# xuanyi-fu/xynet

Measured on AMD Instinct MI355X. Metric: GiB/s device-resident WebSocket XOR-unmask, 64KiB frames, 1/2/4/8 GPUs, higher is better.
Workload: dtype u8; 1 GPU; config 3: 32768 x 64 KiB masked binary frames (H=14), one contiguous 2 GiB batch; decoder=lattice (k_stream_lattice), mode=fused (xyws_decode_stream: boundaries discovered on device), frames_per_gpu=32768, batch_bytes_per_gpu=2147942400, payload_bytes_per_gpu=2147483648, batch_copies=1, parallelism=shard-by-frame x1, no collective

## Files before the change

xynet_amd/csrc/xyws_lattice.h:

```cpp

constexpr uint64_t LAT_FMIN = 128;
constexpr uint64_t LAT_FMAX = 1ull << 40;
enum {
  LW_CNT = 0,
  LW_BRK = 2,
  LW_UNMASK = 3,
  LW_W = 4,
  LW_LOOPS = 5,
  LW_DPOL = 6,
  LW_EPOCH = 7,
  LW_REDIR = 8,
  LW_NBAIL_POL = 12,
  LW_NBAIL_HYP = 13,
  LW_NLOOP_A = 14,
  LW_NLOOP_B = 15,
  LW_RCARRY = 16,
  LW_STAT = 32
};
enum { LS_AGG = 1, LS_BRK = 3 };
constexpr uint32_t LAT_SLIST = 512;
constexpr uint32_t LAT_NOCLAIM = 0x7FFFFFFFu;
enum : uint64_t { RD_DONE = 0, RD_FULL = 1, RD_FROM = 2 };

template <uint32_t NT_, uint32_t SEG_>
struct lgeom {
  static constexpr uint32_t NT = NT_, SEG = SEG_;
  static constexpr uint32_t TMAX = SEG_ / LAT_FMIN + 3;
};
using G_LAT = lgeom<1024, 15 * 8 * 1024>;
using G_LAT5 = lgeom<1024, 15 * 5 * 1024>;
constexpr uint64_t LAT5_MIN_FRAME = 16384;
using G_LAT_SMALL = lgeom<64, 1024>;

static_assert(LW_DPOL == LW_DPOL_WORD && LW_EPOCH == LW_DPOL + 1 && LW_DPOL % 2 == 0, "one 16-byte granule");

template <class GA, class GB>
struct llay {
  static_assert(GA::NT == GB::NT, "one workgroup size");
  static constexpr uint32_t NT = GA::NT;
  static constexpr uint32_t SEG = GA::SEG > GB::SEG ? GA::SEG : GB::SEG;
  static constexpr uint32_t TMAX = GA::TMAX > GB::TMAX ? GA::TMAX : GB::TMAX;
};
template <class GL>
struct __attribute__((aligned(256))) lat_lds {
  cstate S0;
  uint64_t E, X0, F, kmax, c0, kbf, nseg;
  uint64_t gk;
  uint32_t na, cur, nxt, brk, quit, done_last, nsl, big, nogate;
  uint64_t sl_seg[LAT_SLIST], sl_k[LAT_SLIST];
  uint4 tab[GL::TMAX];
  alignas(256) uint8_t seg[GL::SEG + 48];
};

XYWS_DEV uint32_t lat_rel(uint64_t x, uint64_t ss) {
  if (x <= ss) return 0;
  const uint64_t d = x - ss;
  return d > 0xFFFFFFFFull ? 0xFFFFFFFFu : (uint32_t)d;
}

constexpr uint32_t LAT_GRP = 64;
XYWS_DEV uint64_t lat_grp_size(const run_params& P, uint64_t g) {
  const uint64_t a = g * LAT_GRP;
  return a >= P.nseg ? 0 : (P.nseg - a < LAT_GRP ? P.nseg - a : LAT_GRP);
}

XYWS_DEV uint64_t lat_advance(const run_params& P, uint64_t E, uint32_t lane) {
  const uint64_t w = uniform64(st_load(P.lat + LW_W));
  if (w >= P.nseg) return w;
  uint64_t w1 = w;
  {
    const uint64_t g0 = w / LAT_GRP, g = g0 + lane, gs = lat_grp_size(P, g);
    const bool full = !gs || st_load(P.lgrp + g) == gs;
    const uint64_t nf = __ballot(!full);
    const uint32_t c = nf ? (uint32_t)__builtin_ctzll(nf) : 64u;
    const uint64_t wg = (g0 + c) * LAT_GRP;
    if (wg > w1) w1 = wg < P.nseg ? wg : P.nseg;
  }
  if (w1 < P.nseg) {
    bool dec[4];
#pragma unroll
    for (uint32_t r = 0; r < 4; r++) {
      const uint64_t j = w1 + 4 * lane + r;
      dec[r] = j >= P.nseg || (st_load(P.lat + LW_STAT + j) >> 2) == E;
    }
    const uint32_t lc = !dec[0] ? 0u : !dec[1] ? 1u : !dec[2] ? 2u : !dec[3] ? 3u : 4u;
    const uint64_t nd = __ballot(lc < 4);
    uint64_t w2 = w1 + 256;
    if (nd) {
      const uint32_t f = (uint32_t)__builtin_ctzll(nd);
      w2 = w1 + 4 * f + (uint32_t)__shfl((int)lc, (int)f, 64);
    }
    w1 = w2 < P.nseg ? w2 : P.nseg;
  }
  if (w1 > w && lane == 0) __hip_atomic_fetch_max(P.lat + LW_W, w1, __ATOMIC_RELAXED, __HIP_MEMORY_SCOPE_AGENT);
  return w1;
}
XYWS_DEV void lat_wait_decided(const run_params& P, uint64_t E, uint64_t s, uint32_t lane) {
  for (uint32_t it = 0; lat_advance(P, E, lane) <= s; it++) {
    if (it >= (1u << 20)) {
      if (lane == 0) atomicOr(P.head + 1, 2u);
      return;
    }
    __builtin_amdgcn_s_sleep(8);
  }
}

XYWS_DEV u32x4 lat_mask(const uint4* tab, uint32_t nent, uint32_t idx, uint32_t a) {
  const uint4 g = tab[idx];
  if (g.x <= a && a + 16u <= g.y) return u32x4{g.z, g.z, g.z, g.z};
  u32x4 m = span_key16(a, g.x, g.y, g.z);
  if (idx + 1 < nent) {
    const uint4 n = tab[idx + 1];
    if (n.x < a + 16u) m |= span_key16(a, n.x, n.y, n.z);
  }
  return m;
}

XYWS_DEV hdr_info lat_hdr(const run_params& P, const uint8_t* seg, uint32_t xr, uint64_t x) {
  const uint32_t* q = reinterpret_cast<const uint32_t*>(seg + (xr & ~3u));
  const uint32_t sh = xr & 3u, r0 = q[0], r1 = q[1], r2 = q[2], r3 = q[3], r4 = q[4];
  uint32_t w[4];
  w[0] = __builtin_amdgcn_alignbyte(r1, r0, sh);
  w[1] = __builtin_amdgcn_alignbyte(r2, r1, sh);
  w[2] = __builtin_amdgcn_alignbyte(r3, r2, sh);
  w[3] = __builtin_amdgcn_alignbyte(r4, r3, sh);
  const uint64_t room = P.hi - x;
  return parse_header_words(w, room < 16 ? (uint32_t)room : 16u);
}

XYWS_DEV __amdgpu_buffer_rsrc_t lat_rsrc(const run_params& P, uint64_t ss, uint32_t n) {
  const uint64_t top = (P.hi + 15) & ~15ull;
  const uint64_t room = top > ss ? top - ss : 0;
  return __builtin_amdgcn_make_buffer_rsrc(P.base + ss, 0, room < n ? (uint32_t)room : n, 0x00020000);
}

XYWS_DEV void write_frame(const run_params& P, uint64_t ord, uint64_t start, const hdr_info& h, uint64_t ps,
                          int32_t hdr_shift);

XYWS_DEV void lat_carried_frame(const run_params& P, const xyws_carry* cz) {
  if (!P.frames || !P.cap || cz->payload_remaining || !cz->hdr_len) return;
  const hdr_info hh = header_carried(P, cz);
  if (hh.hlen) write_frame(P, 0, P.lo, hh, P.lo + (hh.hlen - cz->hdr_len), (int32_t)cz->hdr_len);
}

template <class LL>
XYWS_DEV void lat_finish(const run_params& P, LL& L) {
  uint64_t* rd = P.lat + LW_REDIR;
  const xyws_carry* cz = P.cin_user ? P.cin_user : &k_zero_carry;
  {
    const uint32_t w = L.na == 2 ? LW_NBAIL_POL : L.na ? LW_NBAIL_HYP : L.big ? LW_NLOOP_A : LW_NLOOP_B;
    st_store(P.lat + w, st_load(P.lat + w) + 1);
  }
  if (L.na) {
    st_store(rd, RD_FULL);
  } else {
    const uint64_t b = st_load(P.lat + LW_BRK);
    const uint64_t X0 = L.X0, F = L.F, kmax = L.kmax, c0 = L.c0;
    lat_carried_frame(P, cz);
    if (b) {
      const uint64_t kb = ~b;
      const uint64_t tb = c0 + kb;
      uint64_t* rc = P.lat + LW_RCARRY;
#pragma unroll
      for (int i = 0; i < 8; i++) st_store(rc + i, 0);
      st_store(rc + 2, cz->frames_total + tb);
      st_store(rd + 1, X0 + kb * F);
      st_store(rd + 2, tb);
      st_store(rd, RD_FROM);
    } else {
      const uint64_t xl = X0 + (kmax - 1) * F;
      const hdr_info h = hdr_global(P, xl, NONE);
      uint64_t total = c0 + kmax;
      cstate S;
      if (!h.hlen) {
        S.X = xl; S.cov_ps = xl; S.cov_start = xl; S.cov_kw = 0; S.cov_key = 0; S.st = S_PARTIAL | S_NOCOV; S.pad = 0;
        total--;
      } else {
        S = frame_state(xl, h);
      }
      xyws_carry cinc;
#pragma unroll
      for (int i = 0; i < 8; i++) reinterpret_cast<uint64_t*>(&cinc)[i] = reinterpret_cast<const uint64_t*>(cz)[i];
      write_outputs(P, &cinc, total, S);
      dpol_publish(P, F, DEC_LATTICE);
      if (P.pol) {
        const uint64_t v[5] = {L.E, P.hi - P.lo, F, F, DEC_LATTICE};
#pragma unroll
        for (int i = 1; i < 5; i++) __hip_atomic_store(P.pol + i, v[i], __ATOMIC_RELAXED, __HIP_MEMORY_SCOPE_SYSTEM);
        __hip_atomic_store(P.pol, v[0], __ATOMIC_RELEASE, __HIP_MEMORY_SCOPE_SYSTEM);
      }
      st_store(rd, RD_DONE);
    }
  }
  uint32_t* cnt = reinterpret_cast<uint32_t*>(P.lat + LW_CNT);
  st_store(P.lat + LW_BRK, 0);
  st_store(P.lat + LW_W, 0);
  st_store(P.lat + LW_LOOPS, 0);
  __hip_atomic_store(cnt, 0u, __ATOMIC_RELAXED, __HIP_MEMORY_SCOPE_AGENT);
  __hip_atomic_store(cnt + 1, 0u, __ATOMIC_RELAXED, __HIP_MEMORY_SCOPE_AGENT);
  st_store(P.lat + LW_EPOCH, L.E);
}

XYWS_DEV bool lat_redirect(run_params& P) {
  if (!(P.opts & XYWS_OPT_REDIRECT)) return true;
  const uint64_t* r = P.lat + LW_REDIR;
  const uint64_t st = uniform64(st_load(r));
  if (st == RD_DONE) return false;
  if (st != RD_FROM) return true;
  const uint64_t p = uniform64(st_load(r + 1)), tb = uniform64(st_load(r + 2));
  const uint64_t pal = p & ~15ull;
  P.obias = p - P.lo;
  P.base += pal;
  P.lo = p - pal;
  P.hi -= pal;
  const uint64_t seg = P.segb, nseg = (P.hi + seg - 1) / seg, maxr = P.nruns;
  P.rbytes = nseg <= maxr ? seg : ((P.hi + maxr - 1) / maxr + 15) & ~15ull;
  P.nruns = (uint32_t)((P.hi + P.rbytes - 1) / P.rbytes);
  P.nflat = 2 * P.nruns;
  P.cin_user = reinterpret_cast<const xyws_carry*>(P.lat + LW_RCARRY);
  P.tbias = tb;
  if (P.frames) {
    const uint64_t c = P.cap < tb ? P.cap : tb;
    P.frames += c;
    P.cap -= c;
  }
  return true;
}

template <class G>
struct lat_io {
  static constexpr bool CTRL = G::NT >= 256;
  static constexpr uint32_t NW = G::NT / 64, NDW = CTRL ? NW - 1 : NW;
  static constexpr uint32_t NROW = G::SEG / 1024, K = (NROW + NDW - 1) / NDW;
  static constexpr uint32_t CLAIM = CTRL ? 64u : 0u;
  static_assert(G::SEG % 1024 == 0, "segments are whole 1 KiB rows");
  XYWS_DEV static bool data_wave(uint32_t wave) { return !CTRL || wave != 0; }
  XYWS_DEV static uint32_t row(uint32_t wave, uint32_t k) { return (CTRL ? wave - 1 : wave) + NDW * k; }
  XYWS_DEV static bool valid(uint32_t wave, uint32_t k) { return K * NDW == NROW || row(wave, k) < NROW; }
};

XYWS_DEV uint64_t lat_load_late(const uint64_t* p) {
  uint64_t v;
  asm volatile("global_load_dwordx2 %0, %1, off sc1" : "=v"(v) : "v"(p) : "memory");
  return v;
}

constexpr uint32_t LAT_NREP = 64, LAT_REPW = 32;
inline constexpr uint64_t lat_rep_off(uint64_t segs) {
  return (LW_STAT + segs + segs / 64 + 1 + LAT_REPW - 1) / LAT_REPW * LAT_REPW;
}
inline constexpr uint64_t lat_sl_off(uint64_t segs) { return lat_rep_off(segs) + LAT_NREP * LAT_REPW; }
XYWS_DEV void lat_raise_brk(const run_params& P, uint64_t k, uint32_t lane) {
  uint64_t o = 0;
  if (lane == 0) o = __hip_atomic_fetch_max(P.lat + LW_BRK, ~k, __ATOMIC_RELAXED, __HIP_MEMORY_SCOPE_AGENT);
  if (uniform64(o) >= ~k) return;
  __hip_atomic_fetch_max(P.lbrk + LAT_REPW * lane, ~k, __ATOMIC_RELAXED, __HIP_MEMORY_SCOPE_AGENT);
  asm volatile("s_waitcnt vmcnt(0)" ::: "memory");
}

XYWS_DEV uint32_t lat_ctrl_load(const run_params& P, uint64_t s, uint64_t SEGB, uint64_t X0, uint64_t F, uint64_t kmax,
                                uint32_t tid) {
  const uint64_t ss = s * SEGB;
  const uint64_t ka = ss <= X0 ? 0 : (ss - X0 + F - 1) / F;
  const uint64_t xc = ka && ka <= kmax ? X0 + (ka - 1) * F : ss;
  const uint64_t top = (P.hi + 3) & ~3ull;
  const uint32_t lane = tid & 63u;
  const bool pd = lane < 4;
  uint64_t q = (pd ? ss + SEGB : xc & ~3ull) + (uint32_t)(pd ? 4u * lane : 4u * (lane - 4u));
  if (q + 4 > top) q = top - 4;
  return __builtin_nontemporal_load(reinterpret_cast<const uint32_t*>(P.base + q));
}

enum { LR_ALL = 0, LR_CTRL = 1, LR_DATA = 2 };
enum { LT_C_A = 16, LT_C_C, LT_C_ADV, LT_D_FILL, LT_D_WB, LT_D_TAB, LT_D_WC, LT_D_MASK, LT_D_WD, LT_D_ST, LT_D_WA,
       LT_SEGS, LT_GATE, LT_END };
struct lat_clock {
  bool on;
  uint64_t t, acc[16];
  XYWS_DEV void start(bool o) {
    on = o;
    for (int i = 0; i < 16; i++) acc[i] = 0;
    t = on ? __builtin_amdgcn_s_memtime() : 0;
  }
  XYWS_DEV void mark(int slot) {
    if (!on) return;
    const uint64_t n = __builtin_amdgcn_s_memtime();
    acc[slot - 16] += n - t;
    t = n;
  }
  XYWS_DEV void flush(const run_params& P) {
    if (!on) return;
    for (int i = 0; i < 16; i++)
      if (acc[i]) stat_add(P, 16 + i, acc[i]);
  }
};
template <class G, int ROLE, class LL>
XYWS_DEV void lat_loop(const run_params& P, LL& L, uint32_t tid0, uint32_t ahead) {
  using IO = lat_io<G>;
  constexpr bool CT = ROLE != LR_DATA, DT = ROLE != LR_CTRL;
  uint32_t tid = tid0;
  asm volatile("" : "+v"(tid));
  const uint32_t lane = tid & 63u;
  const uint32_t wave = __builtin_amdgcn_readfirstlane(tid >> 6);
  uint32_t* cnt = reinterpret_cast<uint32_t*>(P.lat + LW_CNT);
  const uint64_t E = uniform64(L.E);
  const uint64_t X0 = uniform64(L.X0), F = uniform64(L.F), kmax = uniform64(L.kmax);
  const float rF = 1.0f / (float)(F < (1ull << 24) ? F : (1ull << 24));
  const uint32_t F32 = F < 0x80000000ull ? (uint32_t)F : 0x80000000u;
  uint32_t cur = uniform32(L.cur);
  uint32_t it = 0, nsl = 0;
  lat_clock clk;
  clk.start(stats_on(P) && (tid == 0 || (tid == 64 && DT)));
  uint64_t brk_seen = 0;
  const bool cl = tid == 0 && CT;
  u32x4 e[DT ? IO::K : 1];
  uint32_t cx = 0;
  constexpr uint32_t CW = IO::CLAIM / 64u;
  auto issue = [&](uint32_t s, bool claim, bool rows) {
    if constexpr (DT) {
      if (wave == CW) {
        if (lane == 0) {
          if (claim)
            asm volatile("global_atomic_add %0, %1, %2, off sc0" : "=v"(ahead) : "v"(cnt), "v"(1u) : "memory");
          else
            ahead = LAT_NOCLAIM;
        }
        cx = lat_ctrl_load(P, s, G::SEG, X0, F, kmax, tid);
      }
      if (rows) {
        const __amdgpu_buffer_rsrc_t rs = lat_rsrc(P, (uint64_t)s * G::SEG, G::SEG);
#pragma unroll
        for (uint32_t k = 0; k < IO::K; k++)
          e[k] = __builtin_amdgcn_raw_buffer_load_b128(rs, IO::valid(wave, k) ? lane * 16u : OOB,
                                                       IO::row(wave, k) * 1024u, AUX_NT);
      }
    }
  };
  if (DT && cur != NONE32) {
    const uint32_t a0 = ahead;
    issue(cur, false, true);
    ahead = a0;
    const __amdgpu_buffer_rsrc_t rs = lat_rsrc(P, (uint64_t)cur * G::SEG, G::SEG);
#pragma unroll
    for (uint32_t k = 0; k < IO::K; k++)
      __builtin_amdgcn_raw_buffer_store_b128(u32x4{0u, 0u, 0u, 0u}, rs, OOB, k * 1024u, AUX_ST_STREAM);
  }
  const uint32_t dl = IO::CTRL ? tid - 64u : tid, NDL = IO::NDW * 64u;
  while (cur != NONE32) {
    asm volatile("" : "+v"(tid));
    const uint64_t ss = (uint64_t)cur * G::SEG;
    const uint64_t se = ss + G::SEG;
    const uint64_t ka = ss <= X0 ? 0 : (ss - X0 + F - 1) / F;
    clk.mark(cl ? LT_C_ADV : LT_D_ST);
    __syncthreads();
    clk.mark(cl ? LT_C_ADV : LT_D_WA);
    if constexpr (DT) {
#pragma unroll
      for (uint32_t k = 0; k < IO::K; k++)
        if (IO::valid(wave, k)) *reinterpret_cast<u32x4*>(&L.seg[IO::row(wave, k) * 1024u + lane * 16u]) = e[k];
      if (clk.on) asm volatile("s_waitcnt lgkmcnt(0)" ::: "memory");
    }
    if (DT && wave == CW) {
      asm volatile("" : "+v"(ahead), "+v"(cx) : "v"(e[IO::K - 1].x));
      const uint32_t ln = tid & 63u;
      if (ln < 9) *reinterpret_cast<uint32_t*>(&L.seg[G::SEG + 4u * ln]) = cx;
      if (lane == 0) {
        const uint32_t a = ahead + 2u * gridDim.x;
        L.nxt = a < P.nseg ? a : NONE32;
        L.brk = NONE32;
      }
    }
    clk.mark(cl ? LT_C_A : LT_D_FILL);
    __syncthreads();
    clk.mark(cl ? LT_C_A : LT_D_WB);
    const uint32_t nxt = uniform32(L.nxt);
    uint64_t kz = se <= X0 ? 0 : (se - X0 + F - 1) / F;
    if (kz > kmax) kz = kmax;
    const uint32_t nl = kz > ka ? (uint32_t)(kz - ka) : 0u;
    if constexpr (DT) {
      if (tid == IO::CLAIM) {
        uint4 c = {0u, 0u, 0u, 0u};
        if (ka == 0) {
          const cstate S0 = L.S0;
          if (!(S0.st & S_NOCOV)) c = uint4{lat_rel(S0.cov_ps, ss), lat_rel(X0, ss), S0.cov_kw, 0u};
        } else if (ka <= kmax) {
          const uint64_t xc = X0 + (ka - 1) * F;
          const uint32_t sh = (uint32_t)(xc & 3);
          uint32_t w[4];
          const uint32_t* cw = reinterpret_cast<const uint32_t*>(&L.seg[G::SEG + 16]);
#pragma unroll
          for (int i = 0; i < 4; i++) w[i] = __builtin_amdgcn_alignbyte(cw[i + 1], cw[i], sh);
          const uint64_t room = P.hi - xc;
          const hdr_info h = parse_header_words(w, room < 16 ? (uint32_t)room : 16u);
          if (h.hlen) {
            const uint64_t ps = xc + h.hlen;
            const uint64_t end = ka == kmax ? sat_add(ps, h.plen) : xc + F;
            c = uint4{lat_rel(ps, ss), lat_rel(end < P.hi ? end : P.hi, ss), aligned_key(h.key, ps, 0), 0u};
          }
        }
        L.tab[0] = c;
      }
      if (nxt != NONE32) issue(nxt, !L.quit, true);
      const uint32_t nlw = (P.opts & XYWS_OPT_LATX_NOWORK) ? 0u : nl;
      for (uint32_t i = dl; i < nlw; i += NDL) {
        const uint64_t k = ka + i;
        const uint64_t x = X0 + k * F;
        const uint32_t xr = (uint32_t)(x - ss);
        const hdr_info h = lat_hdr(P, L.seg, xr, x);
        const bool last = k + 1 == kmax;
        const uint64_t fend = h.hlen ? sat_add(x + h.hlen, h.plen) : x;
        const bool ok = h.hlen ? ((uint64_t)h.hlen + h.plen == F && h.plen < F) || (last && fend >= P.hi) : last;
        if (!ok) atomicMin(&L.brk, i);
        uint4 en = {xr, xr, 0u, 0u};
        if (h.hlen) {
          const uint64_t ps = x + h.hlen;
          en = uint4{lat_rel(ps, ss), lat_rel(fend < P.hi ? fend : P.hi, ss), aligned_key(h.key, ps, 0), 0u};
        }
        L.tab[1 + i] = en;
      }
    }
    if (CT && tid == 0) {
      asm volatile("s_waitcnt vmcnt(0)" : "+v"(brk_seen)::"memory");
      if (cl) clk.mark(LT_GATE);
      L.gk = brk_seen;
    }
    clk.mark(cl ? LT_C_A : LT_D_TAB);
    __syncthreads();
    clk.mark(cl ? LT_C_C : LT_D_WC);
    const uint32_t brk = uniform32(L.brk);
    const bool blind = (P.opts & XYWS_OPT_TEST_LATSPEC) != 0;
    const bool gate = it == 0 && !blind && !(P.opts & XYWS_OPT_LAT_NOGATE);
    if (CT && tid < 64) {
      const uint64_t gk = uniform64(L.gk);
      if (brk != NONE32 && !(gk && ~gk <= ka + brk)) lat_raise_brk(P, ka + brk, lane);
      if (tid == 0) {
        st_store(P.lat + LW_STAT + cur, (E << 2) | (brk != NONE32 ? LS_BRK : LS_AGG));
        __hip_atomic_fetch_add(P.lgrp + cur / LAT_GRP, 1ull, __ATOMIC_RELAXED, __HIP_MEMORY_SCOPE_AGENT);
      }
      if (gate) {
        const uint64_t tg = clk.on ? __builtin_amdgcn_s_memtime() : 0;
        lat_wait_decided(P, E, cur, lane);
        if (tg && tid == 0) stat_add(P, LT_END, __builtin_amdgcn_s_memtime() - tg);
        if (tid == 0) L.gk = st_load(P.lat + LW_BRK);
      }
      if (tid == 0) brk_seen = lat_load_late(P.lbrk + LAT_REPW * (blockIdx.x % LAT_NREP));
    }
    if (gate) __syncthreads();
    clk.mark(cl ? LT_C_C : LT_D_WD);
    const uint64_t b = blind ? 0 : uniform64(L.gk);
    uint64_t kst = brk != NONE32 ? ka + brk : kz;
    if (b && ~b < kst) kst = ~b;
    uint32_t stop = kst >= kz ? G::SEG : lat_rel(X0 + kst * F, ss);
    if (stop > G::SEG) stop = G::SEG;
    bool quit = b || brk != NONE32;
    if (stop && !gate) {
      if (nsl < LAT_SLIST) {
        if (tid == IO::CLAIM) {
          L.sl_seg[nsl] = cur;
          L.sl_k[nsl] = kst;
        }
        nsl++;
      } else {
        const uint64_t k0 = ka ? ka - 1 : 0;
        if (tid == IO::CLAIM)
          for (uint32_t r = 0; r <= LAT_NREP; r++)
            __hip_atomic_fetch_max(r < LAT_NREP ? P.lbrk + LAT_REPW * r : P.lat + LW_BRK, ~k0, __ATOMIC_RELAXED,
                                   __HIP_MEMORY_SCOPE_AGENT);
        if (k0 < kst) {
          stop = lat_rel(X0 + k0 * F, ss);
          kst = k0;
        }
        quit = true;
      }
    }
    if (quit && tid == IO::CLAIM) L.quit = 1;
    if constexpr (DT) {
      const uint32_t xka = ka < kmax ? lat_rel(X0 + ka * F, ss) : 0xFFFFFFFFu;
      const uint32_t nent = brk != NONE32 ? 1u + brk : 1u + nl;
      const uint32_t lo_r = lat_rel(P.lo, ss), hi_r = P.hi - ss < G::SEG ? (uint32_t)(P.hi - ss) : G::SEG;
      const __amdgpu_buffer_rsrc_t rs = lat_rsrc(P, ss, G::SEG);
      const bool any = !(P.opts & XYWS_OPT_NO_STORE);
      const bool work = !(P.opts & XYWS_OPT_LATX_NOWORK);
      uint32_t edge = 0;
      u32x4 dprev = {0u, 0u, 0u, 0u};
#pragma unroll
      for (uint32_t k = 0; k < IO::K; k++) {
        const bool ok = IO::valid(wave, k);
        const uint32_t a = (ok ? IO::row(wave, k) : 0u) * 1024u + lane * 16u;
        u32x4 d = *reinterpret_cast<const u32x4*>(&L.seg[a]);
        uint32_t idx = 0;
        if (a >= xka) {
          const uint32_t dd = a - xka;
          uint32_t qq = (uint32_t)((float)dd * rF);
          if (qq * F32 > dd) qq--;
          else if ((qq + 1) * F32 <= dd) qq++;
          idx = 1 + qq;
        }
        if (work && idx < nent) d = d ^ lat_mask(L.tab, nent, idx, a);
        const bool whole = ok && a >= lo_r && a + 16u <= hi_r && a + 16u <= stop;
        if (ok && !whole && a < stop && a < hi_r && a + 16u > lo_r) {
          edge |= 1u << k;
          *reinterpret_cast<u32x4*>(&L.seg[a]) = d;
        }
        __builtin_amdgcn_raw_buffer_store_b128(d, rs, (whole && any) ? lane * 16u : OOB, IO::row(wave, k) * 1024u,
                                               AUX_ST_STREAM);
        asm volatile("" ::"v"(dprev.x), "v"(dprev.y), "v"(dprev.z), "v"(dprev.w));
        dprev = d;
      }
      asm volatile("s_nop 1" ::"v"(dprev.x), "v"(dprev.y), "v"(dprev.z), "v"(dprev.w));
#pragma nounroll
      while (edge && any) {
        const uint32_t k = __builtin_ctz(edge);
        edge &= edge - 1;
        const uint32_t a = IO::row(wave, k) * 1024u + lane * 16u;
#pragma nounroll
        for (uint32_t y = a; y < a + 16u; y++)
          if (y >= lo_r && y < hi_r && y < stop) P.base[ss + y] = L.seg[y];
      }
      if (P.frames && stop && kst > ka) {
        const uint32_t nd = (uint32_t)(kst - ka < nl ? kst - ka : nl);
        for (uint32_t i = dl; i < nd; i += NDL) {
          const uint64_t k = ka + i;
          const uint64_t ord = L.c0 + k;
          if (ord >= P.cap) break;
          const uint64_t x = X0 + k * F;
          const hdr_info h = lat_hdr(P, L.seg, (uint32_t)(x - ss), x);
          if (h.hlen) write_frame(P, ord, x, h, x + h.hlen, 0);
        }
      }
    }
    it++;
    if (clk.on && cl) clk.acc[LT_SEGS - 16]++;
    cur = nxt;
  }
  clk.mark(cl ? LT_C_ADV : LT_D_ST);
  clk.flush(P);
  if (DT && tid == IO::CLAIM) L.nsl = nsl;
}

constexpr uint32_t LAT_LSW = 1 + 2 * LAT_SLIST;
template <class G, class LL>
XYWS_DEV void lat_dump_list(const run_params& P, const LL& L, uint32_t tid) {
  const uint32_t n = L.nsl;
  uint64_t* q = P.lsl + (uint64_t)blockIdx.x * LAT_LSW;
  if (tid == 0) q[0] = n;
  for (uint32_t i = tid; i < n; i += G::NT) {
    q[1 + 2 * i] = L.sl_seg[i];
    q[2 + 2 * i] = L.sl_k[i];
  }
}

template <class G, class LL>
XYWS_DEV void lat_undo(const run_params& P, const LL& L, uint32_t tid, uint64_t s, uint64_t kst, uint64_t kb) {
  const uint64_t X0 = L.X0, F = L.F, kmax = L.kmax;
  const uint64_t ss = s * G::SEG;
  const uint32_t stop = (uint32_t)(X0 + kst * F - ss < G::SEG ? X0 + kst * F - ss : G::SEG);
  const uint32_t lo_r = lat_rel(P.lo, ss), hi_r = P.hi - ss < G::SEG ? (uint32_t)(P.hi - ss) : G::SEG;
  const uint32_t top = stop < hi_r ? stop : hi_r;
  const uint32_t from = lat_rel(X0 + kb * F, ss);
  for (uint32_t a = (from & ~15u) + tid * 16u; a < top; a += G::NT * 16u) {
    uint64_t g = a + ss < X0 ? NONE : (a + ss - X0) / F;
    u32x4 m = {0u, 0u, 0u, 0u};
    for (int t = 0; t < 2; t++, g = g == NONE ? 0 : g + 1) {
      uint4 en = {0u, 0u, 0u, 0u};
      if (g == NONE) {
        const cstate S0 = L.S0;
        if (!(S0.st & S_NOCOV)) en = uint4{lat_rel(S0.cov_ps, ss), lat_rel(X0, ss), S0.cov_kw, 0u};
      } else if (g < kst && g < kmax) {
        const uint64_t x = X0 + g * F;
        const hdr_info h = hdr_global(P, x, NONE);
        if (h.hlen) {
          const uint64_t ps = x + h.hlen;
          const uint64_t end = g + 1 == kmax ? sat_add(ps, h.plen) : x + F;
          en = uint4{lat_rel(ps, ss), lat_rel(end < P.hi ? end : P.hi, ss), aligned_key(h.key, ps, 0), 0u};
        }
      }
      m |= span_key16(a, en.x, en.y, en.z);
    }
    if (a >= from && a >= lo_r && a + 16u <= top) {
      uint32_t* q = reinterpret_cast<uint32_t*>(P.base + ss + a);
      const uint32_t mm[4] = {m.x, m.y, m.z, m.w};
#pragma unroll
      for (int i = 0; i < 4; i++) {
        if (!mm[i]) continue;
        const uint32_t v = __hip_atomic_load(q + i, __ATOMIC_RELAXED, __HIP_MEMORY_SCOPE_AGENT);
        __hip_atomic_store(q + i, v ^ mm[i], __ATOMIC_RELAXED, __HIP_MEMORY_SCOPE_AGENT);
      }
      continue;
    }
#pragma unroll
    for (uint32_t b = 0; b < 16; b++) {
      const uint32_t y = a + b;
      const uint32_t mw = b < 4 ? m.x : b < 8 ? m.y : b < 12 ? m.z : m.w;
      const uint8_t kbyte = (uint8_t)(mw >> (8u * (b & 3u)));
      if (kbyte && y >= from && y >= lo_r && y < top) {
        uint8_t* q = P.base + ss + y;
        const uint8_t v = __hip_atomic_load(q, __ATOMIC_RELAXED, __HIP_MEMORY_SCOPE_AGENT);
        __hip_atomic_store(q, (uint8_t)(v ^ kbyte), __ATOMIC_RELAXED, __HIP_MEMORY_SCOPE_AGENT);
      }
    }
  }
}

constexpr uint32_t LAT_UNDO_POLLS = 2048;

template <class G, class LL>
XYWS_DEV void lat_body(const run_params& P, LL& L, uint32_t tid, uint32_t ahead) {
  using IO = lat_io<G>;
  uint32_t* cnt = reinterpret_cast<uint32_t*>(P.lat + LW_CNT);
  if (!L.na) {
    if constexpr (IO::CTRL) {
      if (__builtin_amdgcn_readfirstlane(tid >> 6) == 0)
        lat_loop<G, LR_CTRL>(P, L, tid, ahead);
      else
        lat_loop<G, LR_DATA>(P, L, tid, ahead);
    } else {
      lat_loop<G, LR_ALL>(P, L, tid, ahead);
    }
    __syncthreads();
    if (tid < 64) {
      uint64_t b = 0;
      if (tid == 0) __hip_atomic_fetch_add(P.lat + LW_LOOPS, 1ull, __ATOMIC_RELAXED, __HIP_MEMORY_SCOPE_AGENT);
      if (L.quit && L.nsl) {
        const uint32_t polls = (P.opts & XYWS_OPT_TEST_LATDUMP) ? 0u : LAT_UNDO_POLLS;
        bool ended = false;
        for (uint32_t it = 0; it < polls; it++) {
          if (uniform64(st_load(P.lat + LW_LOOPS)) >= gridDim.x) {
            ended = true;
            break;
          }
          __builtin_amdgcn_s_sleep(8);
        }
        if (ended) b = uniform64(st_load(P.lat + LW_BRK));
      }
      if (tid == 0) L.kbf = b && L.nsl ? ~b : NONE;
    }
    __syncthreads();
    const uint64_t kb = L.kbf;
    if (kb != NONE) {
      const uint32_t n = L.nsl;
      for (uint32_t j = 0; j < n; j++)
        if (kb < L.sl_k[j]) lat_undo<G>(P, L, tid, L.sl_seg[j], L.sl_k[j], kb);
      asm volatile("s_waitcnt vmcnt(0)" ::: "memory");
      __syncthreads();
      if (tid == 0) L.nsl = 0;
      __syncthreads();
    }
    lat_dump_list<G>(P, L, tid);
  }
  asm volatile("s_waitcnt vmcnt(0)" ::: "memory");
  __syncthreads();
  if (tid == 0) {
    __builtin_amdgcn_fence(__ATOMIC_RELEASE, "agent");
    asm volatile("s_waitcnt vmcnt(0)" ::: "memory");
    const uint32_t last = atomicAdd(cnt + 1, 1u) + 1 == gridDim.x ? 1u : 0u;
    if (last) {
      __builtin_amdgcn_fence(__ATOMIC_ACQUIRE, "agent");
      asm volatile("s_waitcnt vmcnt(0)" ::: "memory");
    }
    L.done_last = last;
  }
  __syncthreads();
  if (!L.done_last) return;
  if (tid == 0) {
    const uint64_t b = st_load(P.lat + LW_BRK);
    L.kbf = b && !L.na ? ~b : NONE;
  }
  __syncthreads();
  const uint64_t kb = L.kbf;
  if (kb != NONE) {
    if (tid == 0) L.nsl = 0;
    __syncthreads();
    for (uint32_t w = tid; w < gridDim.x; w += G::NT) {
      const uint64_t* q = P.lsl + (uint64_t)w * LAT_LSW;
      const uint32_t n = (uint32_t)st_load(q);
      for (uint32_t i = 0; i < n; i++) {
        const uint64_t kst = st_load(q + 2 + 2 * i);
        if (kb < kst) {
          const uint32_t j = atomicAdd(&L.nsl, 1u);
          if (j < LAT_SLIST) {
            L.sl_seg[j] = st_load(q + 1 + 2 * i);
            L.sl_k[j] = kst;
          }
        }
      }
    }
    __syncthreads();
    const uint32_t nu = L.nsl;
    if (nu <= LAT_SLIST) {
      for (uint32_t j = 0; j < nu; j++) lat_undo<G>(P, L, tid, L.sl_seg[j], L.sl_k[j], kb);
    } else {
      for (uint32_t w = 0; w < gridDim.x; w++) {
        const uint64_t* q = P.lsl + (uint64_t)w * LAT_LSW;
        const uint32_t n = (uint32_t)st_load(q);
        for (uint32_t i = 0; i < n; i++) {
          const uint64_t kst = st_load(q + 2 + 2 * i);
          if (kb < kst) lat_undo<G>(P, L, tid, st_load(q + 1 + 2 * i), kst, kb);
        }
      }
    }
    asm volatile("s_waitcnt vmcnt(0)" ::: "memory");
    __syncthreads();
  }
  for (uint64_t g = tid; g * LAT_GRP < P.nseg; g += G::NT)
    __hip_atomic_store(P.lgrp + g, 0ull, __ATOMIC_RELAXED, __HIP_MEMORY_SCOPE_AGENT);
  if (tid < LAT_NREP) __hip_atomic_store(P.lbrk + LAT_REPW * tid, 0ull, __ATOMIC_RELAXED, __HIP_MEMORY_SCOPE_AGENT);
  if (tid != 0) return;
  lat_finish(P, L);
}

template <class GA, class GB>
__global__ void __launch_bounds__(GB::NT)
__attribute__((amdgpu_waves_per_eu(GB::NT >= 256 ? GB::NT / 256 : 1))) k_stream_lattice(run_params P0) {
  using GL = llay<GA, GB>;
  using IO = lat_io<GB>;
  static_assert(lat_io<GA>::CLAIM == IO::CLAIM, "one claim lane");
  extern __shared__ __attribute__((aligned(256))) uint8_t xs_lds[];
  lat_lds<GL>& L = *reinterpret_cast<lat_lds<GL>*>(xs_lds);
  const uint32_t tid = threadIdx.x;
  uint32_t ahead = NONE32;
  if (tid == 0) {
    const xyws_carry* cz = P0.cin_user ? P0.cin_user : &k_zero_carry;
    carry_words cc;
    uint32_t r0[5];
    uint64_t dp, ep;
    {
      u32x4 g;
      asm volatile("global_load_dwordx4 %0, %1, off sc1" : "=v"(g) : "v"(P0.lat + LW_DPOL) : "memory");
#pragma unroll
      for (int i = 0; i < 8; i++) cc.w[i] = reinterpret_cast<const uint64_t*>(cz)[i];
      const uint64_t a0 = P0.lo & ~3ull, dl = (P0.hi + 3) & ~3ull;
#pragma unroll
      for (int i = 0; i < 5; i++) {
        const uint64_t q = a0 + 4 * i;
        r0[i] = *reinterpret_cast<const uint32_t*>(P0.base + (q < dl ? q : dl - 4));
      }
      asm volatile("s_waitcnt vmcnt(0)" : "+v"(g)::"memory");
#pragma unroll
      for (int i = 0; i < 5; i++)
        if (a0 + 4 * i >= dl) r0[i] = 0u;
      dp = (uint64_t)g.x | ((uint64_t)g.y << 32);
      ep = (uint64_t)g.z | ((uint64_t)g.w << 32);
    }
    L.E = ep + 1;
    const bool dvalid = dp >> 63, dreg = (dp & ((1ull << 48) - 1)) >= LAT_FMIN;
    const uint64_t ddec = (dp >> 48) & 0x7Fu;
    uint32_t na = dvalid && !dreg && !(P0.opts & XYWS_OPT_LATTICE) ? 2u : 0u;
    L.nogate = dvalid && dreg && ddec == DEC_LATTICE && !(P0.opts & XYWS_OPT_LAT_GATE) ? 1u : 0u;
    uint64_t c0 = 0;
    const cstate S0 = initial_state_w(P0, cc, c0);
    if (!na && ((S0.st & S_PARTIAL) || S0.X >= P0.hi)) na = 1u;
    uint64_t F = 0, kmax = 0;
    if (!na) {
      hdr_info h;
      if (S0.X == P0.lo) {
        const uint32_t sh = (uint32_t)(P0.lo & 3);
        uint32_t w[4];
#pragma unroll
        for (int i = 0; i < 4; i++) w[i] = __builtin_amdgcn_alignbyte(r0[i + 1], r0[i], sh);
        const uint64_t room = P0.hi - P0.lo;
        h = parse_header_words(w, room < 16 ? (uint32_t)room : 16u);
      } else {
        h = hdr_global(P0, S0.X, NONE);
      }
      F = sat_add(h.hlen, h.plen);
      if (!h.hlen || F < LAT_FMIN || F > LAT_FMAX) na = 1;
      else kmax = (P0.hi - S0.X + F - 1) / F;
    }
    if (!na && kmax > 1 && !(P0.opts & (XYWS_OPT_TEST_LATSPEC | XYWS_OPT_LATX_NOCHK))) {
      const uint64_t dl = (P0.hi + 3) & ~3ull;
      uint32_t r[2][5];
#pragma unroll
      for (int j = 0; j < 2; j++) {
        const uint64_t a = (S0.X + (j + 1) * F) & ~3ull;
#pragma unroll
        for (int i = 0; i < 5; i++) {
          const uint64_t q = a + 4 * i;
          r[j][i] = (j == 0 || kmax > 2) && q < dl ? *reinterpret_cast<const uint32_t*>(P0.base + q) : 0u;
        }
      }
#pragma unroll
      for (int j = 0; j < 2; j++) {
        const uint64_t k = j + 1;
        if (k >= kmax) break;
        const uint64_t x = S0.X + k * F;
        const uint32_t sh = (uint32_t)(x & 3);
        uint32_t w[4];
#pragma unroll
        for (int i = 0; i < 4; i++) w[i] = __builtin_amdgcn_alignbyte(r[j][i + 1], r[j][i], sh);
        const uint64_t room = P0.hi - x;
        const hdr_info h = parse_header_words(w, room < 16 ? (uint32_t)room : 16u);
        const bool last = k + 1 == kmax;
        const uint64_t fend = h.hlen ? sat_add(x + h.hlen, h.plen) : x;
        const bool ok = h.hlen ? ((uint64_t)h.hlen + h.plen == F && h.plen < F) || (last && fend >= P0.hi) : last;
        if (!ok) na = 1;
      }
    }
    const bool big = GA::SEG != GB::SEG && !na && F >= LAT5_MIN_FRAME;
    const uint64_t seg = big ? GA::SEG : GB::SEG;
    const uint64_t nseg = (P0.hi + seg - 1) / seg;
    L.nseg = nseg;
    L.S0 = S0;
    L.c0 = c0;
    L.X0 = S0.X;
    L.F = F;
    L.kmax = kmax;
    L.na = na;
    L.quit = 0;
    L.nsl = 0;
    L.big = big ? 1u : 0u;
    L.cur = !na && blockIdx.x < nseg ? blockIdx.x : NONE32;
  }
  if (tid == IO::CLAIM) ahead = blockIdx.x - gridDim.x;
  __syncthreads();
  run_params P = P0;
  P.nseg = uniform64(L.nseg);
  P.opts &= ~XYWS_OPT_LAT_NOGATE;
  if (uniform32(L.nogate)) P.opts |= XYWS_OPT_LAT_NOGATE;
  if constexpr (GA::SEG != GB::SEG) {
    if (uniform32(L.big)) {
      lat_body<GA>(P, L, tid, ahead);
      return;
    }
  }
  lat_body<GB>(P, L, tid, ahead);
}
```

xynet_amd/csrc/xyws_stream.hip:

```cpp
#include <hip/hip_runtime.h>
#include <stdint.h>

#include <cstring>
#include <mutex>
#include <cstdlib>
#include <initializer_list>

#include "xyws_stream.h"
#include "xyws_device.h"

namespace {



constexpr uint64_t NONE = ~0ull;
constexpr uint32_t NONE32 = 0xFFFFFFFFu;
constexpr uint32_t PAD = 32;
constexpr uint32_t KHDR_127 = 2, KHDR_126 = 6, KHDR_7 = 8;
constexpr uint32_t SPIN = 1u << 24;
constexpr uint32_t OOB = 0x80000000u;
constexpr int AUX_NT = 2;
#ifndef XYWS_EXP_AUX_ST
#define XYWS_EXP_AUX_ST 2
#endif
// ... 1504 lines not shown
    }
    if (st_on) stat_add(P, ST_X_SURV, __builtin_amdgcn_s_memtime() - tb);
    (void)check();
  }
  if (!rest && !w0) (void)check();
  if (st_on) {
    stat_add(P, ST_P_TCOMP, a_filt); stat_add(P, ST_P_TCHECK, a_chk);
    stat_add(P, ST_P_WIN, nwin); stat_add(P, ST_P_CAND, nsurv); stat_add(P, ST_P_UND, L.ucnt);
  }
  if (L.ovf) {
    __syncthreads();
    if (tid == 0) L.best = 0xFFFFFFFFu;
    __syncthreads();
#pragma unroll 1
    for (uint32_t k = 0; k < G::CH; k++) {
      const uint32_t a = (k * G::NT + tid) * 16u;
      uint32_t b = ss + a < P.hi ? chunk_candidates<G>(P, L, a, unm) : 0u;
      bool hit = false;
      while (b) {
        const uint32_t t = __builtin_ctz(b);
        b &= b - 1;
        const uint32_t pos = a + t;
        if (pos > __hip_atomic_load(&L.best, __ATOMIC_RELAXED, __HIP_MEMORY_SCOPE_WORKGROUP)) { hit = true; break; }
        if (chain_plausible(P, L, ss, ss + pos, unm, true) == 1u) {
          atomicMin(&L.best, pos);
          hit = true;
          break;
        }
      }
      if (hit) break;
    }
    __syncthreads();
    return;
  }
  const uint32_t nu = L.ucnt, best = L.best;
  if (nu) {
    for (uint32_t i = tid; i < nu; i += G::NT) {
      const uint32_t pos = L.ul[i];
      if (pos < best && chain_plausible(P, L, ss, ss + pos, unm, true) == 1u) atomicMin(&L.best, pos);
    }
    __syncthreads();
    if (st_on) stat_add(P, ST_P_TRES, __builtin_amdgcn_s_memtime() - tq);
  }
}

template <class G>
XYWS_DEV void find_entry(const run_params& P, lds_t<G>& L, seg_io<G>& io, uint32_t tid, uint64_t rb,
                         uint64_t re) {
  const bool unm = (P.opts & XYWS_OPT_UNMASKED_HINT) != 0;
  const bool big = P.bigscan != 0;
  if (re > P.hi) re = P.hi;
  if (tid == 0) L.aux0 = NONE;
  uint64_t tp = (stats_on(P) && tid == 0) ? __builtin_amdgcn_s_memtime() : 0;
  for (uint64_t ss = rb; ss < re; ss += G::SEG) {
    __syncthreads();
    io.fill(P, L, ss, tid);
    if (tid == 0) { L.best = 0xFFFFFFFFu; L.aux1 = ss; }
    __syncthreads();
    if (stats_on(P) && tid == 0) {
      const uint64_t t = __builtin_amdgcn_s_memtime();
      stat_add(P, ST_P_FILL, t - tp);
      tp = t;
    }
    if (ss + G::SEG < P.hi && !(P.opts & XYWS_OPT_DIAG)) io.issue(P, ss + G::SEG, tid);
    if (P.pfs && ss == rb) {
      if (tid == 0) {
        const xyws_carry* cz = P.cin_user ? P.cin_user : &k_zero_carry;
        uint64_t c0;
        const cstate S0 = initial_state(P, cz, c0);
        const uint64_t F = P.pfs, x0 = S0.X;
        if (!(S0.st & (S_PARTIAL | S_PARTCARRY)) && x0 < P.hi) {
          const uint64_t q = rb <= x0 ? x0 : x0 + (rb - x0 + F - 1) / F * F;
          if (q >= ss && q + XYWS_MAX_FRAME_HEADER_SIZE <= ss + G::SEG && q < re) {
            const hdr_info h = hdr_at(P, L, ss, q, NONE);
            if (h.hlen && (uint64_t)h.hlen + h.plen == F && chain_plausible(P, L, ss, q, unm, false) == 1u)
              L.best = (uint32_t)(q - ss);
          }
        }
      }
      __syncthreads();
      if (L.best != 0xFFFFFFFFu) {
        if (tid == 0) {
          L.aux0 = ss + L.best;
          stat_add(P, ST_P_LATTICE, 1);
        }
        break;
      }
    }
    scan_segment<G>(P, L, ss, tid, unm, !big);
    if (stats_on(P) && tid == 0) {
      const uint64_t t = __builtin_amdgcn_s_memtime();
      stat_add(P, ST_P_SCAN, t - tp);
      tp = t;
    }
    if (L.best != 0xFFFFFFFFu) {
      if (tid == 0) L.aux0 = ss + L.best;
      break;
    }
  }
  __syncthreads();
}

template <class G>
XYWS_DEV void prologue(const run_params& P, lds_t<G>& L, seg_io<G>& io, uint32_t tid, uint64_t self, uint64_t rb,
                       uint64_t re) {
  const uint64_t t0 = (stats_on(P) && tid == 0) ? __builtin_amdgcn_s_memtime() : 0;
  find_entry(P, L, io, tid, rb, re);
  const uint64_t tpub = (stats_on(P) && tid == 0) ? __builtin_amdgcn_s_memtime() : 0;
  if (tid == 0) {
    const uint64_t rng_end = re < P.hi ? re : NONE;
    const uint64_t q = L.aux0, ss = L.aux1;
    uint64_t h = NONE, W = NONE, hc = 0;
    cstate S;
    S.X = 0; S.cov_ps = 0; S.cov_start = 0; S.cov_kw = 0; S.cov_key = 0; S.st = S_NOCOV; S.pad = 0;
    if (q != NONE) {
      const hdr_info hq = hdr_at(P, L, ss, q, NONE);
      h = (hq.hlen == 2 || hq.hlen == 6) ? sat_add(q + hq.hlen, hq.plen) : q;
      const hdr_info hh = h < P.hi ? hdr_at(P, L, ss, h, NONE) : hq;
      if (h >= rng_end || h >= P.hi || !hh.hlen) {
        h = NONE;
      } else {
        W = (h + hh.hlen + 15) & ~15ull;
        S = frame_state(h, hh);
        hc = 1;
        record_start<G>(P, L, self, h);
        while (S.X < W && S.X < P.hi) {
          const hdr_info hx = hdr_at(P, L, ss, S.X, NONE);
          if (!hx.hlen) { S.st |= S_PARTIAL; break; }
          record_start<G>(P, L, self, S.X);
          S = frame_state(S.X, hx);
          hc++;
        }
      }
    }
    uint64_t* rec = P.rec + self * R_WORDS;
    st_store(rec + R_H, h);
    st_store(rec + R_W, W);
    put_state(rec + R_S0, S);
    st_store(rec + R_HEAD, hc);
    granule_store(P.flags + 2 * self, flag_published(L.E),
                  (h == NONE ? G_NONE : (h | ((W - h) << 46))) | granule_tag(L.E));
    L.S = S;
    L.cnt = hc;
    L.dense = (h != NONE && S.X - S.cov_start < 1024) ? G::FCAP : 0;
    L.aux2 = h == NONE ? NONE : W;
    stat_add(P, ST_RUNS, 1);
    if (h == NONE) stat_add(P, ST_NONE, 1);
    if (stats_on(P)) stat_add(P, ST_T_PRO, __builtin_amdgcn_s_memtime() - t0);
    if (stats_on(P)) stat_add(P, ST_P_PUB, __builtin_amdgcn_s_memtime() - tpub);
  }
  __syncthreads();
}

XYWS_DEV void write_outputs(const run_params& P, const xyws_carry* cin, uint64_t total, const cstate& o) {
  if (P.nframes) *P.nframes = total + P.tbias;
  __hip_atomic_store(reinterpret_cast<uint64_t*>(P.head + 2), total, __ATOMIC_RELAXED, __HIP_MEMORY_SCOPE_AGENT);
  if (!P.cout) return;
  const uint64_t lo = P.lo, hi = P.hi;
  uint64_t pr = 0, ph = 0, key = 0, hl = 0, h0 = 0, h1 = 0;
  if (o.st & S_PARTIAL) {
    const uint32_t c0 = (o.st & S_PARTCARRY) ? cin->hdr_len : 0u;
    const uint64_t from = (o.st & S_PARTCARRY) ? lo : o.X;
#pragma unroll
    for (uint32_t i = 0; i < XYWS_MAX_FRAME_HEADER_SIZE; i++) {
      uint64_t b = 0;
      bool have = true;
      if (i < c0) b = cin->hdr[i];
      else if (from + (i - c0) < hi) b = P.base[from + (i - c0)];
      else have = false;
      if (have && hl == i) {
        if (i < 8) h0 |= b << (8 * i); else h1 |= b << (8 * (i - 8));
        hl++;
      }
    }
  } else if (o.X > hi && !(o.st & S_NOCOV)) {
    if (o.st & S_CARRIED) {
      pr = cin->payload_remaining - (hi - lo);
      ph = cin->phase + (hi - lo);
      key = (uint64_t)cin->key[0] | ((uint64_t)cin->key[1] << 8) | ((uint64_t)cin->key[2] << 16) |
            ((uint64_t)cin->key[3] << 24);
    } else {
      const hdr_info hh = (o.st & S_HDRCARRY) ? header_carried(P, cin) : hdr_global(P, o.cov_start, NONE);
      pr = hh.plen - (hi - o.cov_ps);
      ph = hi - o.cov_ps;
      key = hh.key;
    }
  }
  uint64_t* c = reinterpret_cast<uint64_t*>(P.cout);
  c[0] = pr;
  c[1] = ph;
  c[2] = cin->frames_total + total;
  c[3] = key | (hl << 32) | (h0 << 40);
  c[4] = (h0 >> 24) | (h1 << 40);
  c[5] = h1 >> 24;
  c[6] = 0;
  c[7] = 0;
}

XYWS_DEV uint64_t entry_of(const run_params& P, uint64_t f) {
  const uint64_t h = st_load(P.rec + f * R_WORDS + R_H);
  const uint64_t sp = st_load(P.rec + (f & ~1ull) * R_WORDS + R_SPLIT);
  return ((f & 1) && sp == NONE) ? NONE : h;
}

template <class G>
XYWS_DEV void finish_fast(const run_params& P, lds_t<G>& L, uint32_t tid) {
  uint64_t* scr = reinterpret_cast<uint64_t*>(L.seg);
  constexpr bool HS_LDS = G::SEG >= 1024 + 16 * MAX_RUNS;
  uint64_t* hs = reinterpret_cast<uint64_t*>(L.seg + 1024);
  const bool one = HS_LDS && P.nflat <= G::NT;
  if (HS_LDS && !one) {
    for (uint32_t r = tid; r < P.nflat; r += G::NT) hs[r] = entry_of(P, r);
  }
  struct rec_t {
    uint64_t h, cw, okw, ep, hn;
    cstate fs;
  };
  auto load_rec = [&](uint32_t r, rec_t& x) {
    const uint64_t* rec = P.rec + (uint64_t)r * R_WORDS;
    x.cw = st_load(rec + R_CNT);
    x.okw = st_load(rec + R_OK);
    x.ep = st_load(rec + R_EP);
    x.hn = st_load(rec + R_HN);
    x.fs = get_state(rec + R_F0);
    x.h = (HS_LDS && !one) ? hs[r] : entry_of(P, r);
  };
  uint64_t c[9];
  if (tid == 0) {
    c[8] = st_load(reinterpret_cast<const uint64_t*>(P.head + HEAD_EPOCH));
#pragma unroll
    for (int i = 0; i < 8; i++) c[i] = st_load(reinterpret_cast<const uint64_t*>(P.cin) + i);
  }
  rec_t x0;
  x0.h = NONE; x0.cw = 0; x0.okw = OK_BIT; x0.ep = 0; x0.hn = NONE;
  if (tid < P.nflat) load_rec(tid, x0);
  if (tid == 0) {
    L.E = c[8] + 1;
#pragma unroll
    for (int i = 0; i < 8; i++) reinterpret_cast<uint64_t*>(&L.cinc)[i] = c[i];
  }
  __syncthreads();
  const uint64_t E = L.E;
  const uint32_t lane = tid & 63u, wave = tid >> 6;
  const bool plan = P.frames && P.cap;
  uint64_t carry = 0;
  uint32_t bad = 0, stale = 0, last = 0;
  bool has = false;
  cstate fsl;
  for (uint32_t t0 = 0; t0 < P.nflat; t0 += G::NT) {
    const uint32_t r = t0 + tid;
    rec_t x;
    if (t0 == 0) {
      x = x0;
    } else {
      x.h = NONE; x.cw = 0; x.okw = OK_BIT; x.ep = E; x.hn = NONE;
      if (r < P.nflat) load_rec(r, x);
    }
    if (r >= P.nflat) x.ep = E;
    if (one) {
      if (r < P.nflat) hs[r] = x.h;
      __syncthreads();
    }
    const uint64_t h = x.h, okw = x.okw, ep = x.ep, hn = x.hn;
    const bool vis = r < P.nflat && (r == 0 || h != NONE);
    const uint64_t cnt = vis ? x.cw : 0;
    if (vis) {
      const uint64_t succ = okw >> 32;
      if (ep != E) stale = 1;
      if (!(okw & OK_BIT) || (okw & TMO_BIT) || ep != E) bad = 1;
      if (succ < P.nflat && hn != (HS_LDS ? hs[succ] : entry_of(P, succ))) bad = 1;
      last = r;
      fsl = x.fs;
      has = true;
    }
    uint64_t xs = cnt;
#pragma unroll
    for (uint32_t o = 1; o < 64; o <<= 1) {
      const uint64_t y = __shfl_up(xs, o, 64);
      if (lane >= o) xs += y;
    }
    if (lane == 63) scr[wave] = xs;
    __syncthreads();
    uint64_t wb = 0, tot = 0;
    for (uint32_t w = 0; w < G::NT / 64; w++) {
      const uint64_t v = scr[w];
      if (w < wave) wb += v;
      tot += v;
    }
    if (vis && plan) {
      uint64_t* rw = P.rec + (uint64_t)r * R_WORDS;
      st_store(rw + R_EFROM, h);
      st_store(rw + R_ECNT, cnt);
      st_store(rw + R_EORD, carry + wb + xs - cnt);
      st_store(rw + R_ECARRY, r == 0 ? 1u : 0u);
    }
    carry += tot;
    __syncthreads();
  }
  if (__syncthreads_or(stale) && tid == 0) atomicOr(P.head + 1, 4u);
  const bool any_bad = __syncthreads_or(bad);
  if (tid == 0) L.aux1 = 0;
  __syncthreads();
  if (last) atomicMax(reinterpret_cast<unsigned long long*>(&L.aux1), (unsigned long long)last);
  __syncthreads();
  if (!any_bad) {
    if (tid == 0) L.aux2 = carry;
    if (has && last == L.aux1) L.S = fsl;
  }
  if (tid == 0) L.act = any_bad ? 1u : 0u;
  __syncthreads();
}

template <class G>
XYWS_DEV void decode_range(const run_params& P, lds_t<G>& L, seg_io<G>& io, uint32_t tid, uint64_t ss0, bool in_lds,
                           uint64_t wlo, uint64_t rng_end, bool victim) {
  if (tid == 0) {
    L.tail = 0; L.past = 0; L.ok = 0; L.done = 0; L.end = 0; L.tmo = 0; L.first_after = NONE;
    L.known = 0;
    L.sgood = P.dense0 ? 0u : 1u;
    L.rng_end = rng_end;
    L.victim = victim ? 1u : 0u;
    L.hn = NONE; L.Wn = NONE; L.succ = P.nflat;
    L.scan_j = L.self + 1;
  }
  __syncthreads();
  const uint64_t t1 = stats_on(P) ? __builtin_amdgcn_s_memtime() : 0;
  run_chain(P, L, io, tid, ss0, in_lds, wlo);
  if (tid == 0) {
    if (L.victim) {
      close_split(P, P.split + 2 * (L.self >> 1), L.E);
      L.victim = 0;
    }
    uint64_t* rec = P.rec + L.self * R_WORDS;
    const bool ok = !L.tmo && (L.succ >= P.nflat || (L.past && L.ok));
    st_store(rec + R_OK, (ok ? OK_BIT : 0) | (L.tmo ? TMO_BIT : 0) | ((uint64_t)L.succ << 32));
// ... 719 lines not shown
```

Baseline: 3076 GiB/s.

## Shorten lattice tail: prefetch last header, fold break flag into completion counter

The last-frame header is now parsed speculatively in the prologue alongside the check loads and cached in LDS. The carry-in copy is also cached in LDS. The grid-completion atomic carries a done flag, so blocks that did not quit skip the release fence, and the break word is read inside the same critical section, removing an extra barrier. The counter increment in lat_finish becomes a single atomic add, and a tail-timing stat is added. The intent is to cut serial latency in the last-block finish path, at the cost of extra prologue loads and more complex completion logic.

```diff
diff --git a/xynet_amd/csrc/xyws_lattice.h b/xynet_amd/csrc/xyws_lattice.h
--- a/xynet_amd/csrc/xyws_lattice.h
+++ b/xynet_amd/csrc/xyws_lattice.h
@@ -47,6 +47,9 @@
   uint64_t E, X0, F, kmax, c0, kbf, nseg;
   uint64_t gk;
   uint32_t na, cur, nxt, brk, quit, done_last, nsl, big, nogate;
+  uint64_t cin[8];
+  hdr_info hl;
+  uint64_t t_tail;
   uint64_t sl_seg[LAT_SLIST], sl_k[LAT_SLIST];
   uint4 tab[GL::TMAX];
   alignas(256) uint8_t seg[GL::SEG + 48];
@@ -143,22 +146,23 @@
   if (hh.hlen) write_frame(P, 0, P.lo, hh, P.lo + (hh.hlen - cz->hdr_len), (int32_t)cz->hdr_len);
 }
 
+constexpr uint32_t LT_TAIL = 30;
+
 template <class LL>
 XYWS_DEV void lat_finish(const run_params& P, LL& L) {
   uint64_t* rd = P.lat + LW_REDIR;
-  const xyws_carry* cz = P.cin_user ? P.cin_user : &k_zero_carry;
+  const xyws_carry* cz = reinterpret_cast<const xyws_carry*>(L.cin);
   {
     const uint32_t w = L.na == 2 ? LW_NBAIL_POL : L.na ? LW_NBAIL_HYP : L.big ? LW_NLOOP_A : LW_NLOOP_B;
-    st_store(P.lat + w, st_load(P.lat + w) + 1);
+    __hip_atomic_fetch_add(P.lat + w, 1ull, __ATOMIC_RELAXED, __HIP_MEMORY_SCOPE_AGENT);
   }
   if (L.na) {
     st_store(rd, RD_FULL);
   } else {
-    const uint64_t b = st_load(P.lat + LW_BRK);
+    const uint64_t kb = L.kbf;
     const uint64_t X0 = L.X0, F = L.F, kmax = L.kmax, c0 = L.c0;
     lat_carried_frame(P, cz);
-    if (b) {
-      const uint64_t kb = ~b;
+    if (kb != NONE) {
       const uint64_t tb = c0 + kb;
       uint64_t* rc = P.lat + LW_RCARRY;
 #pragma unroll
@@ -169,7 +173,7 @@
       st_store(rd, RD_FROM);
     } else {
       const uint64_t xl = X0 + (kmax - 1) * F;
-      const hdr_info h = hdr_global(P, xl, NONE);
+      const hdr_info h = L.hl;
       uint64_t total = c0 + kmax;
       cstate S;
       if (!h.hlen) {
@@ -178,10 +182,7 @@
       } else {
         S = frame_state(xl, h);
       }
-      xyws_carry cinc;
-#pragma unroll
-      for (int i = 0; i < 8; i++) reinterpret_cast<uint64_t*>(&cinc)[i] = reinterpret_cast<const uint64_t*>(cz)[i];
-      write_outputs(P, &cinc, total, S);
+      write_outputs(P, cz, total, S, &h);
       dpol_publish(P, F, DEC_LATTICE);
       if (P.pol) {
         const uint64_t v[5] = {L.E, P.hi - P.lo, F, F, DEC_LATTICE};
@@ -199,6 +200,10 @@
   __hip_atomic_store(cnt, 0u, __ATOMIC_RELAXED, __HIP_MEMORY_SCOPE_AGENT);
   __hip_atomic_store(cnt + 1, 0u, __ATOMIC_RELAXED, __HIP_MEMORY_SCOPE_AGENT);
   st_store(P.lat + LW_EPOCH, L.E);
+  if (stats_on(P)) {
+    asm volatile("s_waitcnt vmcnt(0)" ::: "memory");
+    stat_add(P, LT_TAIL, __builtin_amdgcn_s_memtime() - L.t_tail);
+  }
 }
 
 XYWS_DEV bool lat_redirect(run_params& P) {
@@ -274,6 +279,7 @@
 enum { LR_ALL = 0, LR_CTRL = 1, LR_DATA = 2 };
 enum { LT_C_A = 16, LT_C_C, LT_C_ADV, LT_D_FILL, LT_D_WB, LT_D_TAB, LT_D_WC, LT_D_MASK, LT_D_WD, LT_D_ST, LT_D_WA,
        LT_SEGS, LT_GATE, LT_END };
+static_assert(LT_END + 1 == LT_TAIL, "the stats words of a lattice call");
 struct lat_clock {
   bool on;
   uint64_t t, acc[16];
@@ -515,7 +521,8 @@
         const uint32_t a = IO::row(wave, k) * 1024u + lane * 16u;
 #pragma nounroll
         for (uint32_t y = a; y < a + 16u; y++)
-          if (y >= lo_r && y < hi_r && y < stop) P.base[ss + y] = L.seg[y];
+          if (y >= lo_r && y < hi_r && y < stop)
+            __hip_atomic_store(P.base + ss + y, L.seg[y], __ATOMIC_RELAXED, __HIP_MEMORY_SCOPE_AGENT);
       }
       if (P.frames && stop && kst > ka) {
         const uint32_t nd = (uint32_t)(kst - ka < nl ? kst - ka : nl);
@@ -543,10 +550,10 @@
 XYWS_DEV void lat_dump_list(const run_params& P, const LL& L, uint32_t tid) {
   const uint32_t n = L.nsl;
   uint64_t* q = P.lsl + (uint64_t)blockIdx.x * LAT_LSW;
-  if (tid == 0) q[0] = n;
+  if (tid == 0) st_store(q, n);
   for (uint32_t i = tid; i < n; i += G::NT) {
-    q[1 + 2 * i] = L.sl_seg[i];
-    q[2 + 2 * i] = L.sl_k[i];
+    st_store(q + 1 + 2 * i, L.sl_seg[i]);
+    st_store(q + 2 + 2 * i, L.sl_k[i]);
   }
 }
 
@@ -603,11 +610,13 @@
 }
 
 constexpr uint32_t LAT_UNDO_POLLS = 2048;
+constexpr uint32_t LAT_DONE_FLAG = 1u << 16;
 
 template <class G, class LL>
 XYWS_DEV void lat_body(const run_params& P, LL& L, uint32_t tid, uint32_t ahead) {
   using IO = lat_io<G>;
   uint32_t* cnt = reinterpret_cast<uint32_t*>(P.lat + LW_CNT);
+  uint32_t flag = 0;
   if (!L.na) {
     if constexpr (IO::CTRL) {
       if (__builtin_amdgcn_readfirstlane(tid >> 6) == 0)
@@ -617,6 +626,7 @@
     } else {
       lat_loop<G, LR_ALL>(P, L, tid, ahead);
     }
+    if (tid == 0 && stats_on(P)) L.t_tail = __builtin_amdgcn_s_memtime();
     __syncthreads();
     if (tid < 64) {
       uint64_t b = 0;
@@ -647,26 +657,31 @@
       __syncthreads();
     }
     lat_dump_list<G>(P, L, tid);
+    if (tid == 0 && L.quit) flag = LAT_DONE_FLAG;
+  } else if (tid == 0 && stats_on(P)) {
+    L.t_tail = __builtin_amdgcn_s_memtime();
   }
   asm volatile("s_waitcnt vmcnt(0)" ::: "memory");
   __syncthreads();
   if (tid == 0) {
-    __builtin_amdgcn_fence(__ATOMIC_RELEASE, "agent");
-    asm volatile("s_waitcnt vmcnt(0)" ::: "memory");
-    const uint32_t last = atomicAdd(cnt + 1, 1u) + 1 == gridDim.x ? 1u : 0u;
-    if (last) {
+    if (flag) {
+      __builtin_amdgcn_fence(__ATOMIC_RELEASE, "agent");
+      asm volatile("s_waitcnt vmcnt(0)" ::: "memory");
+    }
+    const uint32_t sum = atomicAdd(cnt + 1, 1u + flag) + 1u + flag;
+    const uint32_t last = (sum & (LAT_DONE_FLAG - 1u)) == gridDim.x ? 1u : 0u;
+    uint64_t kbf = NONE;
+    if (last && sum >= LAT_DONE_FLAG) {
       __builtin_amdgcn_fence(__ATOMIC_ACQUIRE, "agent");
       asm volatile("s_waitcnt vmcnt(0)" ::: "memory");
-    }
+      const uint64_t b = st_load(P.lat + LW_BRK);
+      if (b && !L.na) kbf = ~b;
+    }
+    if (last) L.kbf = kbf;
     L.done_last = last;
   }
   __syncthreads();
   if (!L.done_last) return;
-  if (tid == 0) {
-    const uint64_t b = st_load(P.lat + LW_BRK);
-    L.kbf = b && !L.na ? ~b : NONE;
-  }
-  __syncthreads();
   const uint64_t kb = L.kbf;
   if (kb != NONE) {
     if (tid == 0) L.nsl = 0;
@@ -742,6 +757,8 @@
       dp = (uint64_t)g.x | ((uint64_t)g.y << 32);
       ep = (uint64_t)g.z | ((uint64_t)g.w << 32);
     }
+#pragma unroll
+    for (int i = 0; i < 8; i++) L.cin[i] = cc.w[i];
     L.E = ep + 1;
     const bool dvalid = dp >> 63, dreg = (dp & ((1ull << 48) - 1)) >= LAT_FMIN;
     const uint64_t ddec = (dp >> 48) & 0x7Fu;
@@ -766,23 +783,36 @@
       F = sat_add(h.hlen, h.plen);
       if (!h.hlen || F < LAT_FMIN || F > LAT_FMAX) na = 1;
       else kmax = (P0.hi - S0.X + F - 1) / F;
-    }
-    if (!na && kmax > 1 && !(P0.opts & (XYWS_OPT_TEST_LATSPEC | XYWS_OPT_LATX_NOCHK))) {
+      L.hl = h;
+    }
+    if (!na && kmax > 1) {
+      const bool chk = !(P0.opts & (XYWS_OPT_TEST_LATSPEC | XYWS_OPT_LATX_NOCHK));
       const uint64_t dl = (P0.hi + 3) & ~3ull;
-      uint32_t r[2][5];
-#pragma unroll
-      for (int j = 0; j < 2; j++) {
-        const uint64_t a = (S0.X + (j + 1) * F) & ~3ull;
+      uint32_t r[3][5];
+#pragma unroll
+      for (int j = 0; j < 3; j++) {
+        const uint64_t k = j < 2 ? (uint64_t)j + 1 : kmax - 1;
+        const uint64_t a = (S0.X + k * F) & ~3ull;
+        const bool want = j == 2 || (chk && k < kmax);
 #pragma unroll
         for (int i = 0; i < 5; i++) {
           const uint64_t q = a + 4 * i;
-          r[j][i] = (j == 0 || kmax > 2) && q < dl ? *reinterpret_cast<const uint32_t*>(P0.base + q) : 0u;
-        }
+          r[j][i] = want && q < dl ? *reinterpret_cast<const uint32_t*>(P0.base + q) : 0u;
+        }
+      }
+      {
+        const uint64_t x = S0.X + (kmax - 1) * F;
+        const uint32_t sh = (uint32_t)(x & 3);
+        uint32_t w[4];
+#pragma unroll
+        for (int i = 0; i < 4; i++) w[i] = __builtin_amdgcn_alignbyte(r[2][i + 1], r[2][i], sh);
+        const uint64_t room = P0.hi - x;
+        L.hl = parse_header_words(w, room < 16 ? (uint32_t)room : 16u);
       }
 #pragma unroll
       for (int j = 0; j < 2; j++) {
         const uint64_t k = j + 1;
-        if (k >= kmax) break;
+        if (!chk || k >= kmax) break;
         const uint64_t x = S0.X + k * F;
         const uint32_t sh = (uint32_t)(x & 3);
         uint32_t w[4];
diff --git a/xynet_amd/csrc/xyws_stream.hip b/xynet_amd/csrc/xyws_stream.hip
--- a/xynet_amd/csrc/xyws_stream.hip
+++ b/xynet_amd/csrc/xyws_stream.hip
@@ -1680,7 +1680,8 @@
   __syncthreads();
 }
 
-XYWS_DEV void write_outputs(const run_params& P, const xyws_carry* cin, uint64_t total, const cstate& o) {
+XYWS_DEV void write_outputs(const run_params& P, const xyws_carry* cin, uint64_t total, const cstate& o,
+                            const hdr_info* hc = nullptr) {
   if (P.nframes) *P.nframes = total + P.tbias;
   __hip_atomic_store(reinterpret_cast<uint64_t*>(P.head + 2), total, __ATOMIC_RELAXED, __HIP_MEMORY_SCOPE_AGENT);
   if (!P.cout) return;
@@ -1708,7 +1709,7 @@
       key = (uint64_t)cin->key[0] | ((uint64_t)cin->key[1] << 8) | ((uint64_t)cin->key[2] << 16) |
             ((uint64_t)cin->key[3] << 24);
     } else {
-      const hdr_info hh = (o.st & S_HDRCARRY) ? header_carried(P, cin) : hdr_global(P, o.cov_start, NONE);
+      const hdr_info hh = (o.st & S_HDRCARRY) ? header_carried(P, cin) : hc ? *hc : hdr_global(P, o.cov_start, NONE);
       pr = hh.plen - (hi - o.cov_ps);
       ph = hi - o.cov_ps;
       key = hh.key;
```

Result: no change. 3094 GiB/s, median of 6 (+0.6%).
